# DINT-NSDI24/DINT

Hardware: AMD Instinct MI355X
Metric: Mtxn/s + p50/p99 batch latency, TATP (higher is better)
Workload: dtype u64

## Files before the change

### dint_amd/csrc/dint_bins.h

```cpp
#pragma once
#include <cstdlib>

#include "dint_kernels.h"

#define KV_TB 1024u
#define KV_NONE 0xFFFFFFFFu

__device__ static inline uint32_t block_hash_insert(uint32_t *keys, uint32_t k) {
  uint32_t h = (k * 0x9E3779B1u) >> (32 - 11);
  for (;;) {
    const uint32_t old = atomicCAS(&keys[h], KV_NONE, k);
    if (old == KV_NONE || old == k) return h;
    h = (h + 1) & (2 * KV_TB - 1);
  }
}
static_assert(KV_TB == 1024, "block_hash_insert assumes 2048 slots");

#define KV_PLACE_GRID 64u
__device__ static inline void
kv_scan_place_body(const uint32_t *__restrict__ bin_cnt, uint32_t *bin_off, const uint32_t *__restrict__ big,
                   uint32_t *__restrict__ big_next, uint32_t *__restrict__ blk_pub_next, uint32_t *tail,
                   dint_dev_stats *__restrict__ stats, const uint4 *__restrict__ ovl, uint64_t *__restrict__ ovf) {
  __shared__ uint32_t Sw[KV_TB / 64];
  const uint32_t t = threadIdx.x, lane = t & 63, wave = t >> 6;
  const bool first = blockIdx.x == 0;
  if (first) {
    if (t < 4) big_next[t] = 0;
    blk_pub_next[t] = 0;
    if (t == 0 && tail) tail[0] = tail[1];
  }
  const uint32_t nbig = big[0], novl = big[1];
  if (nbig == 0) return;
  uint32_t run = 0;
  for (uint32_t lo = 0; lo < nbig; lo += KV_TB) {
    const uint32_t bin = lo + t < nbig ? big[4 + lo + t] : KV_NONE;
    const uint32_t extra = bin != KV_NONE ? bin_cnt[bin] - DINT_KV_BINCAP : 0;
    uint32_t tot, x = wave_excl_scan_u32(extra, &tot);
    __syncthreads();
    if (lane == 0) Sw[wave] = tot;
    __syncthreads();
    uint32_t all = 0;
    for (uint32_t w = 0; w < KV_TB / 64; w++) {
      if (w < wave) x += Sw[w];
      all += Sw[w];
    }
    if (bin != KV_NONE) bin_off[bin] = run + x;
    run += all;
  }
  if (first && t == 0) atomicAdd(&stats->big_bin_requests, (unsigned long long)run + (unsigned long long)nbig * DINT_KV_BINCAP);
  __builtin_amdgcn_fence(__ATOMIC_SEQ_CST, "workgroup");
  __syncthreads();
  for (uint32_t i = blockIdx.x * KV_TB + t; i < novl; i += KV_PLACE_GRID * KV_TB) {
    const uint4 o = ovl[i];
    const uint32_t off = __hip_atomic_load(&bin_off[o.z], __ATOMIC_RELAXED, __HIP_MEMORY_SCOPE_WORKGROUP);
    ovf[off + o.w - DINT_KV_BINCAP] = ((uint64_t)o.y << 32) | o.x;
  }
}
static __global__ void __launch_bounds__(KV_TB)
k_kv_scan_place(const uint32_t *__restrict__ bin_cnt, uint32_t *bin_off, const uint32_t *__restrict__ big,
                uint32_t *__restrict__ big_next, uint32_t *__restrict__ blk_pub_next, uint32_t *tail,
                dint_dev_stats *__restrict__ stats, const uint4 *__restrict__ ovl, uint64_t *__restrict__ ovf) {
  kv_scan_place_body(bin_cnt, bin_off, big, big_next, blk_pub_next, tail, stats, ovl, ovf);
}

#define KVB_T 512u
#define KVB_W (KVB_T / 64u)
#define KVB_GRID 512u
#define KVB_NMAX 4096u
#define KVB_NW (KVB_NMAX / 64u)
#define KVB_NBK 2048u
#define KVB_HOT_MIN 256u
#define KVB_HOT_MIN_LOCKS 256u
#define KVB_MMAX 1024u
static_assert(KVB_NW == 64, "the per-word tables are built with one lane per mask word");
static inline uint32_t dint_hot_min(const char *env, uint32_t dflt) {
  const char *v = getenv(env);
  return v && *v ? (uint32_t)strtoul(v, nullptr, 10) : dflt;
}
struct kvb_lead { uint32_t found_link, slot, ver0, la0, lb0; };
struct kvb_carry { uint32_t la, lb, ver; int src; uint32_t miss; };
struct kvb_pop { uint16_t below[KVB_NW + 1]; };
struct kvb_edge { int16_t last[KVB_NW], next[KVB_NW]; };

__device__ static inline void kvb_build_pop(const uint64_t *M, kvb_pop &P) {
  const uint32_t lane = lane_id();
  uint32_t tot;
  const uint32_t x = wave_excl_scan_u32((uint32_t)__popcll(M[lane]), &tot);
  P.below[lane] = (uint16_t)x;
  if (lane == 63) P.below[KVB_NW] = (uint16_t)tot;
}
__device__ static inline void kvb_build_edge(const uint64_t *M, kvb_edge &E) {
  const int lane = (int)lane_id();
  const uint64_t m = M[lane];
  int hi = m ? lane * 64 + 63 - __clzll((long long)m) : -1;
  int lo = m ? lane * 64 + __ffsll((unsigned long long)m) - 1 : 0x7FFF;
#pragma unroll
  for (int d = 1; d < 64; d <<= 1) {
    const int a = __shfl_up(hi, d, 64), b = __shfl_down(lo, d, 64);
    if (lane >= d) hi = max(hi, a);
    if (lane + d < 64) lo = min(lo, b);
  }
  const int a = __shfl_up(hi, 1, 64), b = __shfl_down(lo, 1, 64);
  E.last[lane] = (int16_t)(lane ? a : -1);
  E.next[lane] = (int16_t)((lane == 63 || b == 0x7FFF) ? -1 : b);
}
__device__ static inline bool kvb_bit(const uint64_t *M, uint32_t p) { return (M[p >> 6] >> (p & 63)) & 1ull; }
__device__ static inline uint32_t kvb_below(const uint64_t *M, const kvb_pop &P, uint32_t x) {
  const uint32_t w = x >> 6, r = x & 63;
  return P.below[w] + (r ? (uint32_t)__popcll(M[w] & ((1ull << r) - 1ull)) : 0u);
}
__device__ static inline uint32_t kvb_popc(const uint64_t *M, const kvb_pop &P, uint32_t a, uint32_t b) {
  return a < b ? kvb_below(M, P, b) - kvb_below(M, P, a) : 0u;
}
__device__ static inline int kvb_last(const uint64_t *M, const kvb_edge &E, uint32_t a, uint32_t b) {
  if (a >= b) return -1;
  const uint32_t w = (b - 1) >> 6, r = b & 63;
  const uint64_t m = M[w] & (r ? (1ull << r) - 1ull : ~0ull);
  const int res = m ? (int)(w * 64 + 63 - __clzll((long long)m)) : (int)E.last[w];
  return res >= (int)a ? res : -1;
}
__device__ static inline int kvb_first(const uint64_t *M, const kvb_edge &E, uint32_t a) {
  if (a >= KVB_NMAX) return -1;
  const uint32_t w = a >> 6;
  const uint64_t m = M[w] & (~0ull << (a & 63));
  return m ? (int)(w * 64 + __ffsll((unsigned long long)m) - 1) : (int)E.next[w];
}
__device__ static inline uint32_t kvb_range_popc(const uint64_t *M, uint32_t a, uint32_t b) {
  uint32_t cnt = 0;
  for (uint32_t w = a >> 6; w <= ((b - 1) >> 6) && a < b; w++) {
    uint64_t m = M[w];
    if (w == (a >> 6)) m &= ~0ull << (a & 63);
    if (w == ((b - 1) >> 6) && (b & 63)) m &= (1ull << (b & 63)) - 1ull;
    cnt += (uint32_t)__popcll(m);
  }
  return cnt;
}

__device__ __forceinline__ static uint32_t lane_xor_rt(uint32_t v, uint32_t j) { return (uint32_t)__shfl_xor((int)v, (int)j, 64); }
__device__ __forceinline__ static uint64_t lane_xor_rt(uint64_t v, uint32_t j) {
  return ((uint64_t)lane_xor_rt((uint32_t)(v >> 32), j) << 32) | lane_xor_rt((uint32_t)v, j);
}
#ifdef KVB_SORT_INLINE
#define KVB_SORT_ATTR __forceinline__
#else
#define KVB_SORT_ATTR __attribute__((noinline))
#endif
template <int R, class K>
__device__ KVB_SORT_ATTR static void kvb_sort_blocked_t(K *Sk, uint32_t N) {
// ... 62 lines not shown
```

### dint_amd/csrc/k_kv.hip

```cpp
#include "k_kv_dev.h"

dint_kv_fmt dint_kv_format(uint32_t workload) {
  switch (workload) {
    case DINT_WL_STORE: return {53, 0, 0xFFFFFFFFu, 1, 9, 49, 40};
    case DINT_WL_TATP: return {55, 1, 2, 3, 11, 51, 40};
    default: return {23, 1, 2, 3, 11, 19, 8};
  }
}


static inline uint32_t kv_pick_coarse(uint32_t n, uint32_t load) {
  uint64_t c = ((uint64_t)n + load - 1) / load;
  if (c < 1) c = 1;
  if (c > DINT_KV_CMAX) c = DINT_KV_CMAX;
  return (uint32_t)c;
}
static uint32_t kv_env(const char *name, uint32_t dflt) {
  const char *v = getenv(name);
  return v && *v ? (uint32_t)strtoul(v, nullptr, 10) : dflt;
}
static dint_kv_knobs kv_read_knobs() {
  dint_kv_knobs k;
  k.coarse_load = std::min(8192u, std::max(64u, kv_env("DINT_KV_COARSE_LOAD", KVB_T)));
  k.cap = kv_env("DINT_KV_CAP", 0);
// ... 5 lines not shown
  k.no_split = kv_env("DINT_KV_NO_SPLIT", 0);
  k.split_min = std::max(65u, kv_env("DINT_KV_SPLIT_MIN", 65u));
  k.split_target = std::min(448u, std::max(8u, kv_env("DINT_KV_SPLIT_TARGET", 384u)));
  k.one_big_kernel = kv_env("DINT_KV_ONE_BIG_KERNEL", 0);
  k.no_ahead = kv_env("DINT_KV_NO_AHEAD", 0);
  k.no_fuse = kv_env("DINT_KV_NO_FUSE", 0);
  k.sb_split_min = kv_env("DINT_KV_SB_SPLIT_MIN", 65u);
  k.sb_late_grid = std::max(1u, std::min(KVB_GRID, kv_env("DINT_KV_SB_LATE_GRID", 32u)));
  k.sb_npmax = std::max(2u, std::min(KSB_NPMAX, kv_env("DINT_KV_SB_NPMAX", 128u)));
  k.sb_workers = kv_env("DINT_KV_SB_WORKERS", k.sb_npmax + 2u);
  if (k.sb_workers) k.sb_workers = std::max(k.sb_workers, k.sb_npmax + 2u);
  k.workers = std::min(1024u, std::max(KVR_NPMAX + 2u, kv_env("DINT_KV_WORKERS", KVW_GRID)));
  k.part_first = kv_env("DINT_KV_PART_FIRST", 0) & 1u;
  k.late_grid = std::min(KVB_GRID, std::max(1u, kv_env("DINT_KV_LATE_GRID", 8u)));
  k.late_big = kv_env("DINT_KV_LATE_BIG", 0);
  k.exp_no_late = kv_env("DINT_EXP_NO_LATE", 0);
  k.late_fat = kv_env("DINT_KV_LATE_FAT", 0);
  return k;
}

static inline bool kv_uses_hot(const dint_kv &kv, int load_mode) {
  return kv.workload != DINT_WL_SMALLBANK && !(kv.force_rounds & 3) && !load_mode && !kv.knobs.no_split;
}
bool dint_kv_one_launch(const dint_kv &kv, int load_mode) {
  return kv_uses_hot(kv, load_mode) && !kv.knobs.one_big_kernel && !kv.knobs.no_fuse;
}
bool dint_kv_ahead_ok(const dint_kv &kv, int load_mode) {
  if (kv.workload == DINT_WL_SMALLBANK) return !load_mode && !kv.knobs.no_ahead && !kv.knobs.no_fuse;
  return kv_uses_hot(kv, load_mode) && !kv.knobs.one_big_kernel && !kv.knobs.no_ahead;
}

static void kv_fill_pass(kv_pass_args &A, const void *d_req, void *d_rep, uint32_t n, const dint_kv &kv, dint_log log,
                         const dint_scratch &s, int load_mode, const dint_view &view, uint32_t tile) {
  const dint_kv_knobs &K = kv.knobs;
  const uint32_t C = kv_pick_coarse(n, K.coarse_load);
  const uint32_t mean = (n + C - 1) / C;
  uint32_t cap = K.cap_mult * mean + 64;
  cap = std::min(cap, (uint32_t)(s.kbins_slots / C));
  cap = std::max(1u, K.cap ? std::min(cap, K.cap) : cap);
  A.req = (const uint8_t *)d_req; A.rep = (uint8_t *)d_rep; A.n = n;
  A.n_tiles = (n + tile - 1) / tile;
  A.kv = kv.d_dev; A.log = log; A.cut = kv_make_cut(C, n); A.cap = cap;
  A.lcap = K.lcap;
  const uint64_t pn = s.kvs.pass_no;
  A.pno = (uint32_t)(pn & 1u);
  A.bin_cnt = s.kvs.bin_cnt[pn & 1]; A.kbins = s.kvs.kbins[pn & 1]; A.ovl = s.kvs.ovl[pn & 1];
  A.big = s.kvs.ctl[pn % 3]; A.big_z = s.kvs.ctl[(pn + 2) % 3];
  A.blk_pub = s.kvs.pub[pn % 3]; A.blk_pub_z = s.kvs.pub[(pn + 2) % 3];
  A.bigrdy = s.kvs.bigrdy;
  A.ovf = s.ovf; A.ovf2 = s.ovf2; A.stats = s.stats;
  A.bigq = s.bigq;
  A.hotpub = s.hotpub;
  A.lateq = s.lateq;
  A.seq = s.pass_seq ? s.pass_seq : 1u;
  A.inv_n = n > 1 ? (uint32_t)((1ull << 32) / n) : 0xFFFFFFFFu;
  A.load_mode = load_mode;
  A.force_flags = kv.force_rounds | (K.no_bm ? 4 : 0) | (int)(K.hot_min << 8);
  A.split_min = kv_uses_hot(kv, load_mode) ? K.split_min : 0xFFFFFFFFu;
  A.split_target = K.split_target;
  A.np_max = KVR_NPMAX;
  A.sb_pieces = 0;
  A.sbx = s.kvs.sbx;
  if (kv.workload == DINT_WL_SMALLBANK && K.sb_split_min && s.kvs.sbx && !(kv.force_rounds & 3) && !load_mode && !K.no_split) {
    A.split_min = std::max(8u, K.sb_split_min);
    A.np_max = K.sb_npmax;
    A.sb_pieces = 1;
  }
  A.has_log = kv.workload != DINT_WL_STORE;
  A.trace = kv.d_trace;
  A.V = view;
}

extern template int kv_piece_residency<DINT_WL_STORE>(int);
extern template int kv_piece_residency<DINT_WL_TATP>(int);
extern template int kv_piece_residency<DINT_WL_SMALLBANK>(int);
extern template void launch_kv_passes<DINT_WL_STORE>(kv_multi_args &, uint32_t, uint32_t, hipStream_t, hipEvent_t *, const dint_kv_knobs &, bool, const kv_multi_args *, uint32_t);
extern template void launch_kv_passes<DINT_WL_TATP>(kv_multi_args &, uint32_t, uint32_t, hipStream_t, hipEvent_t *, const dint_kv_knobs &, bool, const kv_multi_args *, uint32_t);
extern template void launch_kv_passes<DINT_WL_SMALLBANK>(kv_multi_args &, uint32_t, uint32_t, hipStream_t, hipEvent_t *, const dint_kv_knobs &, bool, const kv_multi_args *, uint32_t);

static inline uint32_t kv_pick_rpt(uint32_t n_total, const dint_kv_knobs &K) {
  if (K.rpt == 1 || K.rpt == 2 || K.rpt == 4) return K.rpt;
  return n_total >= 1024u * 1024u ? 4u : n_total >= 256u * 1024u ? 2u : 1u;
}
static inline uint32_t kv_pick_rpt_ahead(uint32_t n, const dint_kv_knobs &K) {
  if (K.rpt == 4 || (K.rpt == 0 && n >= 256u * 1024u)) return 4u;
  return 2u;
}

static void launch_kv_dispatch(uint32_t workload, kv_multi_args &M, uint32_t n_eng, uint32_t rpt, hipStream_t st, hipEvent_t *ev,
                               const dint_kv_knobs &K, bool part_done = false, const kv_multi_args *next = nullptr, uint32_t next_rpt = 0) {
  switch (workload) {
    case DINT_WL_STORE: launch_kv_passes<DINT_WL_STORE>(M, n_eng, rpt, st, ev, K, part_done, next, next_rpt); break;
    case DINT_WL_TATP: launch_kv_passes<DINT_WL_TATP>(M, n_eng, rpt, st, ev, K, part_done, next, next_rpt); break;
    default: launch_kv_passes<DINT_WL_SMALLBANK>(M, n_eng, rpt, st, ev, K, part_done, next, next_rpt); break;
  }
}

void dint_launch_kv(const void *d_req, void *d_rep, uint32_t n, const dint_kv &kv, dint_log log, dint_scratch s,
                    int load_mode, hipStream_t st, hipEvent_t *ev, const dint_view &view, bool part_done, const dint_kv_ahead *next) {
  if (n == 0) return;
  kv_multi_args M;
  memset(&M, 0, sizeof M);
  const uint32_t rpt = kv_pick_rpt(n, kv.knobs), rpt_a = kv_pick_rpt_ahead(n, kv.knobs);
  kv_fill_pass(M.e[0], d_req, d_rep, n, kv, log, s, load_mode, view, part_done ? KVB_T * rpt_a : KV_TB * rpt);
  kv_multi_args N;
  uint32_t next_rpt = 0;
  if (next && next->n && dint_kv_ahead_ok(kv, load_mode)) {
    dint_scratch sn = s;
    sn.kvs.pass_no = s.kvs.pass_no + 1;
    sn.pass_seq = s.pass_seq + 1 >= 0x3FFFFFFFu ? 1u : s.pass_seq + 1;
    next_rpt = kv_pick_rpt_ahead(next->n, kv.knobs);
    memset(&N, 0, sizeof N);
    kv_fill_pass(N.e[0], next->d_req, next->d_rep, next->n, kv, log, sn, load_mode, next->view, KVB_T * next_rpt);
  } else {
    next = nullptr;
  }
  launch_kv_dispatch(kv.workload, M, 1, rpt, st, ev, kv.knobs, part_done, next ? &N : nullptr, next_rpt);
}

void dint_launch_kv_multi(const dint_kv_pass *p, uint32_t n_eng, hipStream_t st, bool part_done, const dint_kv_pass *next) {
  if (n_eng == 0) return;
  kv_multi_args M, N;
  memset(&M, 0, sizeof M);
  uint32_t n_total = 0;
  for (uint32_t k = 0; k < n_eng; k++) n_total += p[k].n;
  const uint32_t rpt = kv_pick_rpt(n_total, p[0].kv->knobs);
  for (uint32_t k = 0; k < n_eng; k++) kv_fill_pass(M.e[k], p[k].d_req, p[k].d_rep, p[k].n, *p[k].kv, p[k].log, p[k].s, 0, p[k].view, KV_TB * rpt);
  uint32_t next_rpt = 0;
  if (next) {
    uint32_t nmax = 0;
    for (uint32_t k = 0; k < n_eng; k++) nmax = std::max(nmax, next[k].n);
    next_rpt = kv_pick_rpt_ahead(nmax, p[0].kv->knobs);
    memset(&N, 0, sizeof N);
    for (uint32_t k = 0; k < n_eng; k++) {
      dint_scratch sn = next[k].s;
      sn.kvs.pass_no = p[k].s.kvs.pass_no + 1;
      sn.pass_seq = p[k].s.pass_seq + 1 >= 0x3FFFFFFFu ? 1u : p[k].s.pass_seq + 1;
      kv_fill_pass(N.e[k], next[k].d_req, next[k].d_rep, next[k].n, *next[k].kv, next[k].log, sn, 0, next[k].view, KVB_T * next_rpt);
    }
  }
  launch_kv_dispatch(p[0].kv->workload, M, n_eng, rpt, st, nullptr, p[0].kv->knobs, part_done, next ? &N : nullptr, next_rpt);
}
bool dint_kv_multi_ahead_ok(const dint_kv &kv) { return dint_kv_ahead_ok(kv, 0) && !kv.knobs.no_fuse; }

__global__ void __launch_bounds__(256)
k_home_kv(const uint8_t *__restrict__ req, uint32_t n, const kv_dev *__restrict__ kv, dint_kv_fmt f,
          uint8_t *__restrict__ home) {
  const uint32_t i = blockIdx.x * 256u + threadIdx.x;
  if (i >= n) return;
  const uint8_t *m = req + (size_t)i * f.msg;
  const uint32_t table = f.table == 0xFFFFFFFFu ? 0 : m[f.table];
  if (table >= kv->n_tables) { home[i] = 0xFF; return; }
  const uint64_t g = dint_fastmod(dint_hash_key(ld_u64(m + f.key)), kv->mod[table]);
  home[i] = (uint8_t)(g % (kv->shard_count ? kv->shard_count : 1));
}
void dint_launch_home_kv(const void *d_req, uint32_t n, const dint_kv &kv, uint8_t *d_home, hipStream_t st) {
  if (n == 0) return;
  hipLaunchKernelGGL(k_home_kv, dim3((n + 255) / 256), dim3(256), 0, st, (const uint8_t *)d_req, n, kv.d_dev,
                     dint_kv_format(kv.workload), d_home);
}

int dint_kv_create(dint_kv *kv, uint32_t workload, uint64_t n_rows, dint_shard shard, uint32_t pool_entries,
                   uint32_t flags) {
  *kv = dint_kv();
  kv->workload = workload;
  kv->h.same_key = (workload == DINT_WL_TATP && (flags & DINT_FLAG_LOCK_SAME_KEY)) ? 1 : 0;
  uint64_t hs[DINT_KV_MAX_TABLES] = {0, 0, 0, 0, 0};
  if (workload == DINT_WL_STORE) {
// ... 206 lines not shown
```

### dint_amd/csrc/k_kv_dev.h

```cpp
#pragma once
#include <algorithm>
#include <cstdlib>
#include <cstring>
#include <utility>
#include <vector>

#include "../../include/dint_abi.h"
#include "dint_kv.h"
#define KVB_SORT_INLINE
#include "dint_bins.h"

template <int WL> struct Fmt;
template <> struct Fmt<DINT_WL_STORE> {
  static constexpr uint32_t MSG = 53, TYPE = 0, KEY = 1, VAL = 9, VER = 49, VS = 40;
  static constexpr bool HAS_TABLE = false;
  static constexpr uint32_t TABLE = 0;
};
template <> struct Fmt<DINT_WL_TATP> {
  static constexpr uint32_t MSG = 55, TYPE = 1, KEY = 3, VAL = 11, VER = 51, VS = 40;
  static constexpr bool HAS_TABLE = true;
  static constexpr uint32_t TABLE = 2;
};
template <> struct Fmt<DINT_WL_SMALLBANK> {
  static constexpr uint32_t MSG = 23, TYPE = 1, KEY = 3, VAL = 11, VER = 19, VS = 8;
// ... 69 lines not shown
  uint32_t q = __umulhi(gk, c.magic), r = gk - q * c.P;
  if (r >= c.P) { r -= c.P; q++; }
  *bin = r;
  return q;
}
__device__ static inline uint32_t kv_cut_gk(uint32_t gq, uint32_t bin, const kv_cut &c) { return gq * c.P + bin; }
__device__ static inline uint64_t kv_rec(uint32_t gq, uint32_t idx, uint32_t pay, const kv_cut &c) {
  return ((uint64_t)gq << (16 + c.ibits)) | ((uint64_t)idx << 16) | (pay & 0xFFFFu);
}
__device__ static inline uint32_t kv_rec_pay(uint64_t r) { return (uint32_t)r & 0xFFFFu; }
__device__ static inline uint32_t kv_rec_idx(uint64_t r, const kv_cut &c) { return (uint32_t)(r >> 16) & (uint32_t)((1ull << c.ibits) - 1ull); }
__device__ static inline uint64_t kv_sort_key(uint64_t r, const kv_cut &c) {
  const uint32_t pay = kv_rec_pay(r);
  return ((r >> (16 + c.ibits)) << (16 + c.ibits)) | ((uint64_t)((pay >> 7) & 511u) << (7 + c.ibits)) |
         ((uint64_t)kv_rec_idx(r, c) << 7) | (pay & 0x7Fu);
}

struct kv_reqinfo {
  uint32_t type, table, cls;
  uint64_t key;
};
template <int WL>
__device__ static inline kv_reqinfo kv_read_request(const uint8_t *m, bool live, const kv_dev *kv, int load_mode) {
  using F = Fmt<WL>;
  kv_reqinfo r = {0, 0, 0, 0};
  if (live) {
    r.type = m[F::TYPE];
    r.table = F::HAS_TABLE ? m[F::TABLE] : 0;
    r.cls = kv_class<WL>(r.type, load_mode);
    if (r.table >= kv->n_tables) r.cls = 0;
    if (r.cls) r.key = ld_u64(m + F::KEY);
  }
  return r;
}

struct kv_pass_args {
  const uint8_t *req;
  uint8_t *rep;
  uint32_t n, n_tiles;
  const kv_dev *kv;
  dint_log log;
  kv_cut cut;
  uint32_t cap;
  uint32_t lcap;
  uint32_t *bin_cnt;
  uint4 *kbins;
  uint32_t *big, *big_z;
  uint32_t *blk_pub, *blk_pub_z;
  uint32_t *bigrdy;
  uint64_t *sbx;
  uint32_t np_max;
  uint32_t sb_pieces;
  uint32_t pno;
  uint4 *ovl;
  uint64_t *ovf;
  uint64_t *ovf2;
  uint4 *bigq;
  unsigned long long *hotpub;
  uint4 *lateq;
  uint32_t split_min;
  uint32_t split_target;
  uint32_t inv_n;
  uint32_t seq;
  dint_dev_stats *stats;
  int load_mode, force_flags;
  uint32_t has_log;
  uint64_t *trace;
  dint_view V;
};
struct kv_multi_args { kv_pass_args e[DINT_KV_MULTI_MAX]; };

__device__ static inline uint64_t u4_key(const uint4 &r) { return ((uint64_t)r.y << 32) | r.x; }
__device__ static inline uint64_t u4_meta(const uint4 &r) { return ((uint64_t)r.w << 32) | r.z; }

template <uint32_t TB, uint32_t... Ks>
__device__ __forceinline__ static void kv_copy_tile(const uint4 *__restrict__ s, uint4 *__restrict__ d, uint32_t nv, uint32_t t,
                                                    std::integer_sequence<uint32_t, Ks...>) {
  const uint4 v[] = {s[min(t + Ks * TB, nv - 1)]...};
  ((d[min(t + Ks * TB, nv - 1)] = v[Ks]), ...);
}

template <int RPT, uint32_t TB = KV_TB>
struct kv_part_lds {
  uint32_t Hc[DINT_KV_CMAX];
  uint32_t Sov[2];
  uint32_t Stile;
  uint32_t Swl[TB / 64 * RPT], Swp[TB / 64];
};
template <int WL, int RPT, uint32_t TB = KV_TB>
__device__ __forceinline__ static void kv_part_body(const kv_pass_args &A, kv_part_lds<RPT, TB> &S, bool first_block) {
  using F = Fmt<WL>;
  constexpr uint32_t T = TB * RPT, NWV = TB / 64;
  auto &Hc = S.Hc; auto &Sov = S.Sov; auto &Stile = S.Stile; auto &Swl = S.Swl; auto &Swp = S.Swp;
  const uint32_t t = threadIdx.x, lane = t & 63, wv = t >> 6;
  const uint32_t n = A.n, C = A.cut.P;
  const kv_dev *__restrict__ kv = A.kv;
  const uint8_t *__restrict__ req = A.req;
  uint8_t *rep = A.rep;
  if (t == 0) { Stile = atomicAdd(&A.big[2], 1u); Sov[0] = 0; }
  for (uint32_t k = t; k < C; k += TB) Hc[k] = 0;
  __syncthreads();
  const uint32_t tile = Stile;
  kv_reqinfo r[RPT];
  size_t moff[RPT];
  uint64_t lm[RPT];
  uint32_t idx[RPT];
#pragma unroll
  for (int j = 0; j < RPT; j++) {
    idx[j] = tile * T + (uint32_t)j * TB + t;
    bool live;
    moff[j] = dint_view_off(A.V, idx[j] < n ? idx[j] : 0, F::MSG, &live);
    live = live && idx[j] < n;
    r[j] = kv_read_request<WL>(req + moff[j], live, kv, A.load_mode);
    lm[j] = __ballot(r[j].cls == 2);
    if (live && !r[j].cls) atomicAdd(&A.stats->bad_requests, 1ULL);
  }
  if (WL != DINT_WL_STORE) {
    if (lane == 0) {
#pragma unroll
      for (int j = 0; j < RPT; j++) Swl[j * NWV + wv] = (uint32_t)__popcll(lm[j]);
    }
    __syncthreads();
    if (t == 0) {
      uint32_t c = 0;
      for (uint32_t w = 0; w < NWV * RPT; w++) c += Swl[w];
      __hip_atomic_store(&A.blk_pub[tile], 0x80000000u | c, __ATOMIC_RELAXED, __HIP_MEMORY_SCOPE_AGENT);
    }
  }
  if (rep != req) {
    const size_t lo = (size_t)tile * T * F::MSG;
    const size_t hi = min((size_t)n * F::MSG, lo + (size_t)T * F::MSG);
    if ((((uintptr_t)req | (uintptr_t)rep) & 15) == 0) {
      constexpr uint32_t K = (T * F::MSG / 16 + TB - 1) / TB;
      const uint32_t nv = (uint32_t)((hi - lo) / 16);
      const uint4 *s = (const uint4 *)(req + lo);
      uint4 *d = (uint4 *)(rep + lo);
      if (nv) kv_copy_tile<TB>(s, d, nv, t, std::make_integer_sequence<uint32_t, K>());
      for (size_t k = lo + (size_t)nv * 16 + t; k < hi; k += TB) rep[k] = req[k];
    } else {
      for (size_t k = lo + t; k < hi; k += TB) rep[k] = req[k];
    }
  }

  uint32_t coarse[RPT], mypos[RPT];
  uint64_t meta[RPT];
#pragma unroll
  for (int j = 0; j < RPT; j++) {
    coarse[j] = KV_NONE; mypos[j] = 0; meta[j] = 0;
    if (r[j].cls == 1) {
      const uint64_t h = dint_hash_key(r[j].key);
      const uint64_t g = dint_fastmod(h, kv->mod[r[j].table]);
      uint32_t local = (uint32_t)g;
      bool mine = true;
      if (kv->shard_count > 1) {
        mine = (uint32_t)(g % kv->shard_count) == kv->shard_index;
        if (!mine && !A.load_mode) atomicAdd(&A.stats->foreign_requests, 1ULL);
        local = (uint32_t)(g / kv->shard_count);
      }
      if (mine) {
        const uint64_t hs = kv->mod[r[j].table].d, dq = dint_fastmod(h, kv->lockmod[r[j].table]) - g;
        const uint32_t q = dq >= 2 * hs ? (dq >= 3 * hs ? 3u : 2u) : (dq >= hs ? 1u : 0u);
        const uint32_t gq = kv_cut_div(kv->gk_base[r[j].table] + local, A.cut, &coarse[j]);
        meta[j] = kv_rec(gq, idx[j], kv_pay(r[j].type, q, (uint32_t)(h >> 40) & 511u), A.cut);
        mypos[j] = atomicAdd(&Hc[coarse[j]], 1u);
      }
    }
  }
  __syncthreads();
  for (uint32_t c = t; c < C; c += TB) {
    const uint32_t cnt = Hc[c];
    if (cnt) Hc[c] = atomicAdd(&A.bin_cnt[c], cnt);
  }
  __syncthreads();
  uint32_t orank[RPT];
  bool over[RPT];
#pragma unroll
  for (int j = 0; j < RPT; j++) {
    over[j] = false; orank[j] = 0;
    if (coarse[j] != KV_NONE) {
      const uint32_t pos = Hc[coarse[j]] + mypos[j];
      if (pos < A.cap) {
        A.kbins[(size_t)coarse[j] * A.cap + pos] = make_uint4((uint32_t)r[j].key, (uint32_t)(r[j].key >> 32), (uint32_t)meta[j], (uint32_t)(meta[j] >> 32));
      } else {
        over[j] = true;
        orank[j] = atomicAdd(&Sov[0], 1u);
      }
    }
  }
  __syncthreads();
  if (Sov[0]) {
    if (t == 0) Sov[1] = atomicAdd(&A.big[1], Sov[0]);
    __syncthreads();
#pragma unroll
    for (int j = 0; j < RPT; j++)
      if (over[j]) {
        uint4 *o = A.ovl + 2 * (size_t)(Sov[1] + orank[j]);
        o[0] = make_uint4((uint32_t)r[j].key, (uint32_t)(r[j].key >> 32), (uint32_t)meta[j], (uint32_t)(meta[j] >> 32));
        o[1] = make_uint4(coarse[j], 0u, 0u, 0u);
      }
  }

  if (WL != DINT_WL_STORE) {
    const dint_log log = A.log;
    uint32_t part = 0;
    for (uint32_t k = t; k < tile; k += TB) {
      uint32_t v;
      do { v = __hip_atomic_load(&A.blk_pub[k], __ATOMIC_RELAXED, __HIP_MEMORY_SCOPE_AGENT); } while (!(v >> 31));
      part += v & 0x7FFFFFFFu;
    }
    uint32_t tot;
    wave_excl_scan_u32(part, &tot);
    if (lane == 0) Swp[wv] = tot;
    __syncthreads();
    uint32_t base = 0, tile_total = 0;
    for (uint32_t w = 0; w < NWV; w++) base += Swp[w];
    for (uint32_t w = 0; w < NWV * RPT; w++) tile_total += Swl[w];
    const uint32_t tw = A.pno & 1u;
    if (tile == A.n_tiles - 1 && t == 0) {
      const uint32_t total = base + tile_total;
      log.tail[tw ^ 1u] = (uint32_t)(((uint64_t)log.tail[tw] + total) % log.cap);
      *(unsigned long long *)(log.tail + 2) += total;
    }
#pragma unroll
    for (int j = 0; j < RPT; j++) {
      if (r[j].cls != 2) continue;
      uint32_t pos_in_batch = base + (uint32_t)__popcll(lm[j] & lanemask_lt());
      for (uint32_t w = 0; w < (uint32_t)j * NWV + wv; w++) pos_in_batch += Swl[w];
      const uint32_t pos = (uint32_t)(((uint64_t)log.tail[tw] + pos_in_batch) % log.cap);
      uint8_t *e8 = log.ring + (size_t)pos * 64;
      const uint8_t *m = req + moff[j];
      const uint32_t ver = ld_u32(m + F::VER);
      uint8_t *rp = rep + moff[j];
      if (WL == DINT_WL_TATP && r[j].type == 24) {
        *(uint64_t *)e8 = r[j].key;
        *(uint2 *)(e8 + 48) = make_uint2(ver, 1u | (r[j].table << 8));
        rp[F::TYPE] = 27;
      } else {
        const uint8_t *v8 = m + F::VAL;
        uint4 *e4 = (uint4 *)e8;
        e4[0] = make_uint4((uint32_t)r[j].key, (uint32_t)(r[j].key >> 32), ld_u32(v8), ld_u32(v8 + 4));
        if (F::VS == 40) {
          e4[1] = make_uint4(ld_u32(v8 + 8), ld_u32(v8 + 12), ld_u32(v8 + 16), ld_u32(v8 + 20));
          e4[2] = make_uint4(ld_u32(v8 + 24), ld_u32(v8 + 28), ld_u32(v8 + 32), ld_u32(v8 + 36));
        }
        *(uint2 *)(e8 + 48) = make_uint2(ver, r[j].table << 8);
        rp[F::TYPE] = (WL == DINT_WL_TATP) ? 17 : 15;
      }
    }
  }
  if (first_block && t < KV_NLISTS)
    for (uint32_t k = 0; k < kv->n_tables; k++) kv_pool_rotate<kv_dev_mem>(kv->tab[k], t, (A.pno & 1u) * KV_NLISTS);
}

template <int WL, int RPT>
__global__ void __launch_bounds__(KV_TB) k_kv_part(kv_multi_args M) {
  const kv_pass_args &A = M.e[blockIdx.y];
  if (blockIdx.x >= A.n_tiles) return;
  __shared__ kv_part_lds<RPT> S;
  kv_part_body<WL, RPT>(A, S, blockIdx.x == 0);
}

__device__ static inline void kv_stamp(uint64_t *tr, uint32_t k) {
  if (tr) {
    asm volatile("s_waitcnt vmcnt(0) lgkmcnt(0)" ::: "memory");
    if (lane_id() == 0) tr[k] = __builtin_amdgcn_s_memrealtime();
  }
}
__device__ static inline void kv_stamp_real(uint64_t *tr, uint32_t k) {
  if (tr && lane_id() == 0) tr[k] = __builtin_amdgcn_s_memrealtime();
}

#define KV_POOL_MARGIN 4096u
__device__ static inline uint32_t kv_pool_low(const kv_tab &t) {
  return __hip_atomic_load(t.pool_top, __ATOMIC_RELAXED, __HIP_MEMORY_SCOPE_AGENT) + KV_POOL_MARGIN >= t.pool_cap;
}

template <int WL>
__device__ static inline void kv_do_request(uint8_t *msg, uint32_t type, uint32_t table, uint32_t q, uint64_t bucket,
                                            const kv_dev *kv, dint_dev_stats *__restrict__ stats) {
  using F = Fmt<WL>;
  const kv_tab t = kv->tab[table];
  uint8_t *ie = kv_entry_ptr(t, bucket, KV_INLINE);
  kv_hdr H;
  kv_hdr_load(H, ie);
  uint2 cnt = make_uint2(0, 0);
  if (WL == DINT_WL_SMALLBANK) cnt = *(const uint2 *)(ie + KV_SB_LOCK_OFF + 8 * q);
  const uint64_t key = ld_u64(msg + F::KEY);
  uint8_t *val = msg + F::VAL;

  uint32_t act = KV_ACT_NONE, code = 0, ins_ver = 0;
  bool miss_counts = false;
  int lock_store = -1;
  bool cnt_store = false;
  if (type == DINT_KV_LOAD_OP) {
    act = KV_ACT_INS;
    ins_ver = ld_u32(msg + F::VER);
  } else if (WL == DINT_WL_STORE) {
    switch (type) {
      case 0: act = KV_ACT_GET; break;
      case 1: act = KV_ACT_SET; break;
      default: act = KV_ACT_INS; code = 8; break;
    }
  } else if (WL == DINT_WL_TATP) {
    const uint32_t lk = (H.lockw >> (8 * q)) & 0xFFu;
    switch (type) {
      case 0: act = KV_ACT_GET; break;
      case 1:
        if (lk == 0) { lock_store = 1; code = 7; }
        else code = (kv->same_key && *(const uint64_t *)(ie + KV_OWNER_OFF + 8 * q) == key) ? 28 : 8;
        break;
      case 2: lock_store = 0; code = 9; break;
      case 12: act = KV_ACT_SET; miss_counts = true; lock_store = 0; code = 15; break;
      case 18: act = KV_ACT_INS; lock_store = 0; code = 20; break;
      case 22: act = KV_ACT_DEL; miss_counts = true; lock_store = 0; code = 25; break;
      case 13: act = KV_ACT_SET; miss_counts = true; code = 16; break;
      case 19: act = KV_ACT_INS; code = 21; break;
      default: act = KV_ACT_DEL; miss_counts = true; code = 26; break;
    }
    if (lock_store >= 0 && (uint32_t)lock_store == lk) lock_store = -1;
  } else {
    switch (type) {
      case 0: if (cnt.x == 0) { cnt.y++; cnt_store = true; act = KV_ACT_GET; miss_counts = true; code = 7; } else code = 8; break;
      case 1: if (cnt.x == 0 && cnt.y == 0) { cnt.x++; cnt_store = true; act = KV_ACT_GET; miss_counts = true; code = 9; } else code = 10; break;
      case 2: cnt.y--; cnt_store = true; code = 11; break;
      case 3: cnt.x--; cnt_store = true; code = 12; break;
      case 4: act = KV_ACT_SET; miss_counts = true; code = 13; break;
      case 17: act = KV_ACT_GET; code = 18; break;
      default: act = KV_ACT_SET; miss_counts = true; code = 14; break;
// ... 3129 lines not shown
  const uint32_t t = threadIdx.x;
  if (t < sizeof(kv_dev) / 4) ((uint32_t *)&Skv)[t] = ((const uint32_t *)A.kv)[t];
  __syncthreads();
  kv_dev_pend_set(Skv, A.pno);
  __syncthreads();
  kv_cut cut2 = A.cut;
  cut2.P = A.cut.P * KVR_F;
  if (from_late) {
    for (uint32_t i = blockIdx.x; i < nq; i += gridDim.x) {
      const uint4 d = A.lateq[i];
      const uint64_t *recs = (d.w ? (const uint64_t *)A.ovf2 : A.ovf) + d.y;
      kv_big_bin<WL>(A.rep, A.n, cut2, &Skv, d.x, recs, d.w || !A.ovf2 ? nullptr : A.ovf2 + d.y, d.z, A.stats, A.force_flags, A.V, Lraw, Lbm, nullptr);
    }
    return;
  }
  uint64_t *tr = A.trace ? A.trace + 2048 * 32 + 32 * (size_t)(blockIdx.y * KVB_GRID + blockIdx.x) : nullptr;
  for (bool first = true;; first = false) {
    __syncthreads();
    if (t == 0) Stk = atomicAdd(&A.big[4], 1u);
    __syncthreads();
    const uint32_t i = Stk;
    if (i >= nq) break;
    const uint4 d = A.bigq[KVQ_W * (size_t)i];
    uint32_t src = 0, off = d.y, cnt = d.z;
    uint64_t *ttr = first ? tr : nullptr;
    if (ttr && t == 0) { ttr[0] = __builtin_amdgcn_s_memrealtime(); ttr[2] = d.z; ttr[3] = d.x; ttr[30] = d.w; }
    const uint64_t t_in = tr ? __builtin_amdgcn_s_memrealtime() : 0ull;
    int run = 1;
    if ((d.w & 3u) == KVQ_SOLO && WL != DINT_WL_SMALLBANK)
      run = kv_solo_item<WL>(A.rep, cut2, &Skv, d, A.ovf, A.ovf2, A.stats, A.force_flags & 1, A.V, Lraw, &src, &off, &cnt, ttr);
    else if ((d.w & 3u) != KVQ_SUB && WL == DINT_WL_SMALLBANK)
      run = kv_sb_item<WL>(A.rep, cut2, &Skv, d, A.bigq[KVQ_W * (size_t)i + 1], A.bigq[KVQ_W * (size_t)i + 2], A.ovf, A.ovf2, A.hotpub, A.sbx, A.seq,
                           A.inv_n, A.stats, A.V, Lraw, &src, &off, &cnt);
    else if ((d.w & 3u) != KVQ_SUB)
      run = kv_hot_item<WL>(A.rep, cut2, &Skv, d, A.bigq[KVQ_W * (size_t)i + 1], A.bigq[KVQ_W * (size_t)i + 2], A.ovf, A.ovf2, A.hotpub, A.seq,
                            A.inv_n, A.stats, A.force_flags & 1, A.V, Lraw, &src, &off, &cnt, ttr);
    if (run) {
      const uint64_t *recs = (src ? (const uint64_t *)A.ovf2 : A.ovf) + off;
      kv_big_bin<WL>(A.rep, A.n, cut2, &Skv, d.x, recs, src || !A.ovf2 ? nullptr : A.ovf2 + off, cnt, A.stats, A.force_flags, A.V, Lraw, Lbm, ttr);
    }
    if (ttr && t == 0) ttr[1] = __builtin_amdgcn_s_memrealtime();
    if (tr && t == 0) {
      const uint64_t dt = __builtin_amdgcn_s_memrealtime() - t_in;
      if (dt > (tr[31] >> 40)) tr[31] = (dt << 40) | ((uint64_t)(d.z & 0xFFFFFu) << 20) | (d.w & 0x3FFFFu) | (run ? 1ull << 18 : 0ull);
    }
  }
}

template <int WL>
int kv_piece_residency(int device) {
  int per_cu = 0, cus = 0;
  hipError_t e1 = WL == DINT_WL_SMALLBANK
                      ? hipOccupancyMaxActiveBlocksPerMultiprocessor(&per_cu, k_kv_big<WL>, (int)KVB_T, 0)
                      : hipOccupancyMaxActiveBlocksPerMultiprocessor(&per_cu, k_kv_pass<WL, 0>, (int)KVB_T, 0);
  hipError_t e2 = hipDeviceGetAttribute(&cus, hipDeviceAttributeMultiprocessorCount, device);
  if (e1 != hipSuccess || e2 != hipSuccess) { (void)hipGetLastError(); return 0; }
  return per_cu * cus;
}

template <int WL>
void launch_kv_passes(kv_multi_args &M, uint32_t n_eng, uint32_t rpt, hipStream_t st, hipEvent_t *ev, const dint_kv_knobs &K,
                      bool part_done, const kv_multi_args *next , uint32_t next_rpt) {
  uint32_t max_tiles = 0, sum_c = 0;
  for (uint32_t k = 0; k < n_eng; k++) {
    max_tiles = std::max(max_tiles, M.e[k].n_tiles);
    sum_c += M.e[k].cut.P;
  }
  if (ev) hipEventRecord(ev[0], st);
  if (part_done) {}
  else if (rpt == 1) hipLaunchKernelGGL((k_kv_part<WL, 1>), dim3(max_tiles, n_eng), dim3(KV_TB), 0, st, M);
  else if (rpt == 2) hipLaunchKernelGGL((k_kv_part<WL, 2>), dim3(max_tiles, n_eng), dim3(KV_TB), 0, st, M);
  else hipLaunchKernelGGL((k_kv_part<WL, 4>), dim3(max_tiles, n_eng), dim3(KV_TB), 0, st, M);
  if (ev) hipEventRecord(ev[1], st);
  const bool hot = WL != DINT_WL_SMALLBANK && M.e[0].split_min != 0xFFFFFFFFu && !K.one_big_kernel;
  bool fused = false, one = false;
  uint32_t sb_workers = 0;
  if constexpr (WL != DINT_WL_SMALLBANK) {
    if (hot && !K.no_fuse) {
      uint32_t nmax = 0;
      for (uint32_t k = 0; next && k < n_eng; k++) nmax = std::max(nmax, next->e[k].n_tiles);
      const dim3 g(sum_c + K.workers * n_eng + nmax * n_eng);
      if (!next) hipLaunchKernelGGL((k_kv_pass<WL, 0>), g, dim3(KVB_T), 0, st, M, n_eng, sum_c, M, 0u, K.workers, K.part_first);
      else if (next_rpt == 2) hipLaunchKernelGGL((k_kv_pass<WL, 2>), g, dim3(KVB_T), 0, st, M, n_eng, sum_c, *next, nmax, K.workers, K.part_first);
      else hipLaunchKernelGGL((k_kv_pass<WL, 4>), g, dim3(KVB_T), 0, st, M, n_eng, sum_c, *next, nmax, K.workers, K.part_first);
      one = fused = true;
    }
  } else {
    sb_workers = !K.no_fuse && !K.one_big_kernel && M.e[0].sb_pieces ? K.sb_workers : 0u;
    if ((next || sb_workers) && !K.no_fuse) {
      uint32_t nmax = 0;
      for (uint32_t k = 0; next && k < n_eng; k++) nmax = std::max(nmax, next->e[k].n_tiles);
      const dim3 g(sum_c + sb_workers * n_eng + nmax * n_eng);
      if (!next) hipLaunchKernelGGL((k_kv_pass<WL, 0>), g, dim3(KVB_T), 0, st, M, n_eng, sum_c, M, 0u, sb_workers, 0u);
      else if (next_rpt == 2) hipLaunchKernelGGL((k_kv_pass<WL, 2>), g, dim3(KVB_T), 0, st, M, n_eng, sum_c, *next, nmax, sb_workers, K.part_first);
      else hipLaunchKernelGGL((k_kv_pass<WL, 4>), g, dim3(KVB_T), 0, st, M, n_eng, sum_c, *next, nmax, sb_workers, K.part_first);
      one = true;
    }
  }
  if (!one) hipLaunchKernelGGL((k_kv_resolve<WL>), dim3(sum_c), dim3(KVB_T), 0, st, M, n_eng);
  const bool ev3 = ev && one && WL != DINT_WL_SMALLBANK;
  if (ev) hipEventRecord(ev[2], st);
  if constexpr (WL != DINT_WL_SMALLBANK) {
    if (hot && next && !one && n_eng == 1) {
      const dim3 g(KVB_GRID + next->e[0].n_tiles);
      if (next_rpt == 2) hipLaunchKernelGGL((k_kv_hot_part<WL, 2>), g, dim3(KVB_T), 0, st, M.e[0], next->e[0]);
      else hipLaunchKernelGGL((k_kv_hot_part<WL, 4>), g, dim3(KVB_T), 0, st, M.e[0], next->e[0]);
      fused = true;
    }
  }
  if (hot && !fused) hipLaunchKernelGGL((k_kv_hot<WL>), dim3(KVB_GRID, n_eng), dim3(KVB_T), 0, st, M);
  if (ev && !ev3) hipEventRecord(ev[3], st);
  if constexpr (WL != DINT_WL_SMALLBANK) {
    if (hot && K.exp_no_late == 1) {}
    else if (hot && !K.late_big) {
      for (uint32_t r = 0; r < std::max(1u, K.exp_no_late >> 1); r++)
        if (K.late_fat) hipLaunchKernelGGL((k_kv_late<WL, 2>), dim3(KVL_GRID, n_eng), dim3(KVB_T), 0, st, M, r);
        else hipLaunchKernelGGL((k_kv_late<WL, 4>), dim3(KVL_GRID, n_eng), dim3(KVB_T), 0, st, M, r);
    }
    else hipLaunchKernelGGL((k_kv_big<WL>), dim3(hot ? K.late_grid : KVB_GRID, n_eng), dim3(KVB_T), 0, st, M, hot ? 1u : 0u);
  } else {
    hipLaunchKernelGGL((k_kv_big<WL>), dim3(sb_workers ? K.sb_late_grid : KVB_GRID, n_eng), dim3(KVB_T), 0, st, M, sb_workers ? 1u : 0u);
  }
  if (ev) hipEventRecord(ev3 ? ev[3] : ev[4], st);
}
```

Measured before the change: 3024.

## Stage partition records in LDS, sort locally by bin, and enlarge look-ahead tiles

Restructures the partition body to stage each request's key and packed metadata in shared memory. The records are counting-sorted by coarse bin within the tile, so the writes to global bins become contiguous runs instead of scattered per-thread stores. The request copy is done per sub-tile, interleaved with parsing, and log-entry positions are prefix-scanned once. The look-ahead partition tile grows to 8 rows per thread, and the threshold for choosing it is lowered. This raises LDS use per block and may reduce occupancy, and the log path now re-reads request bytes.

```diff
diff --git a/dint_amd/csrc/dint_bins.h b/dint_amd/csrc/dint_bins.h
--- a/dint_amd/csrc/dint_bins.h
+++ b/dint_amd/csrc/dint_bins.h
@@ -64,6 +64,9 @@
 }
 
 #define KVB_T 512u
+#ifndef KVP_AHEAD_RPT
+#define KVP_AHEAD_RPT 8
+#endif
 #define KVB_W (KVB_T / 64u)
 #define KVB_GRID 512u
 #define KVB_NMAX 4096u
diff --git a/dint_amd/csrc/k_kv.hip b/dint_amd/csrc/k_kv.hip
--- a/dint_amd/csrc/k_kv.hip
+++ b/dint_amd/csrc/k_kv.hip
@@ -111,8 +111,9 @@
   if (K.rpt == 1 || K.rpt == 2 || K.rpt == 4) return K.rpt;
   return n_total >= 1024u * 1024u ? 4u : n_total >= 256u * 1024u ? 2u : 1u;
 }
+#define KVP_AHEAD_MIN (128u * 1024u)
 static inline uint32_t kv_pick_rpt_ahead(uint32_t n, const dint_kv_knobs &K) {
-  if (K.rpt == 4 || (K.rpt == 0 && n >= 256u * 1024u)) return 4u;
+  if (K.rpt == 4 || (K.rpt == 0 && n >= KVP_AHEAD_MIN)) return KVP_AHEAD_RPT;
   return 2u;
 }
 
diff --git a/dint_amd/csrc/k_kv_dev.h b/dint_amd/csrc/k_kv_dev.h
--- a/dint_amd/csrc/k_kv_dev.h
+++ b/dint_amd/csrc/k_kv_dev.h
@@ -175,122 +175,185 @@
 
 template <int RPT, uint32_t TB = KV_TB>
 struct kv_part_lds {
+  uint4 st[TB * RPT];
   uint32_t Hc[DINT_KV_CMAX];
-  uint32_t Sov[2];
+  uint32_t Sov[3];
   uint32_t Stile;
-  uint32_t Swl[TB / 64 * RPT], Swp[TB / 64];
+  uint32_t Swl[TB / 64 * RPT + 1];
+  uint32_t Swp[TB / 64], Ssc[TB / 64];
 };
+#define KVP_NOREC (~0ull)
 template <int WL, int RPT, uint32_t TB = KV_TB>
 __device__ __forceinline__ static void kv_part_body(const kv_pass_args &A, kv_part_lds<RPT, TB> &S, bool first_block) {
   using F = Fmt<WL>;
-  constexpr uint32_t T = TB * RPT, NWV = TB / 64;
+  constexpr int RS = RPT >= 2 ? 2 : 1;
+  static_assert(RPT % RS == 0, "a tile is whole sub-tiles");
+  constexpr uint32_t T = TB * RPT, TS = TB * RS, NWV = TB / 64, CPT = DINT_KV_CMAX / TB;
+  constexpr uint32_t IB = T <= 1024 ? 10 : T <= 2048 ? 11 : T <= 4096 ? 12 : 13;
+  static_assert(T <= 8192 && DINT_KV_CMAX % TB == 0 && (TS * F::MSG) % 16 == 0, "tile shape");
   auto &Hc = S.Hc; auto &Sov = S.Sov; auto &Stile = S.Stile; auto &Swl = S.Swl; auto &Swp = S.Swp;
   const uint32_t t = threadIdx.x, lane = t & 63, wv = t >> 6;
   const uint32_t n = A.n, C = A.cut.P;
   const kv_dev *__restrict__ kv = A.kv;
   const uint8_t *__restrict__ req = A.req;
   uint8_t *rep = A.rep;
-  if (t == 0) { Stile = atomicAdd(&A.big[2], 1u); Sov[0] = 0; }
+  if (t == 0) { Stile = atomicAdd(&A.big[2], 1u); Sov[0] = 0; Sov[2] = 0; }
   for (uint32_t k = t; k < C; k += TB) Hc[k] = 0;
   __syncthreads();
-  const uint32_t tile = Stile;
-  kv_reqinfo r[RPT];
-  size_t moff[RPT];
+  const uint32_t tile = Stile, i0 = tile * T;
   uint64_t lm[RPT];
-  uint32_t idx[RPT];
-#pragma unroll
-  for (int j = 0; j < RPT; j++) {
-    idx[j] = tile * T + (uint32_t)j * TB + t;
-    bool live;
-    moff[j] = dint_view_off(A.V, idx[j] < n ? idx[j] : 0, F::MSG, &live);
-    live = live && idx[j] < n;
-    r[j] = kv_read_request<WL>(req + moff[j], live, kv, A.load_mode);
-    lm[j] = __ballot(r[j].cls == 2);
-    if (live && !r[j].cls) atomicAdd(&A.stats->bad_requests, 1ULL);
-  }
   if (WL != DINT_WL_STORE) {
-    if (lane == 0) {
-#pragma unroll
-      for (int j = 0; j < RPT; j++) Swl[j * NWV + wv] = (uint32_t)__popcll(lm[j]);
+#pragma unroll
+    for (int j = 0; j < RPT; j++) {
+      const uint32_t idx = i0 + (uint32_t)j * TB + t;
+      bool live;
+      const size_t moff = dint_view_off(A.V, idx < n ? idx : 0, F::MSG, &live);
+      live = live && idx < n;
+      bool islog = false;
+      if (live) {
+        const uint8_t *m = req + moff;
+        const uint32_t table = F::HAS_TABLE ? m[F::TABLE] : 0;
+        islog = kv_class<WL>(m[F::TYPE], A.load_mode) == 2 && table < kv->n_tables;
+      }
+      lm[j] = __ballot(islog);
+      if (lane == 0) Swl[j * NWV + wv] = (uint32_t)__popcll(lm[j]);
     }
     __syncthreads();
     if (t == 0) {
       uint32_t c = 0;
-      for (uint32_t w = 0; w < NWV * RPT; w++) c += Swl[w];
+      for (uint32_t w = 0; w < NWV * RPT; w++) { const uint32_t v = Swl[w]; Swl[w] = c; c += v; }
+      Swl[NWV * RPT] = c;
       __hip_atomic_store(&A.blk_pub[tile], 0x80000000u | c, __ATOMIC_RELAXED, __HIP_MEMORY_SCOPE_AGENT);
     }
   }
-  if (rep != req) {
-    const size_t lo = (size_t)tile * T * F::MSG;
-    const size_t hi = min((size_t)n * F::MSG, lo + (size_t)T * F::MSG);
-    if ((((uintptr_t)req | (uintptr_t)rep) & 15) == 0) {
-      constexpr uint32_t K = (T * F::MSG / 16 + TB - 1) / TB;
-      const uint32_t nv = (uint32_t)((hi - lo) / 16);
-      const uint4 *s = (const uint4 *)(req + lo);
-      uint4 *d = (uint4 *)(rep + lo);
-      if (nv) kv_copy_tile<TB>(s, d, nv, t, std::make_integer_sequence<uint32_t, K>());
-      for (size_t k = lo + (size_t)nv * 16 + t; k < hi; k += TB) rep[k] = req[k];
+#pragma unroll 1
+  for (uint32_t s = 0; s < (uint32_t)(RPT / RS); s++) {
+    if (rep != req) {
+      const size_t lo = ((size_t)i0 + (size_t)s * TS) * F::MSG;
+      const size_t hi = min((size_t)n * F::MSG, lo + (size_t)TS * F::MSG);
+      if (lo < hi) {
+        if ((((uintptr_t)req | (uintptr_t)rep) & 15) == 0) {
+          constexpr uint32_t K = (TS * F::MSG / 16 + TB - 1) / TB;
+          const uint32_t nv = (uint32_t)((hi - lo) / 16);
+          const uint4 *sv = (const uint4 *)(req + lo);
+          uint4 *dv = (uint4 *)(rep + lo);
+          if (nv) kv_copy_tile<TB>(sv, dv, nv, t, std::make_integer_sequence<uint32_t, K>());
+          for (size_t k = lo + (size_t)nv * 16 + t; k < hi; k += TB) rep[k] = req[k];
+        } else {
+          for (size_t k = lo + t; k < hi; k += TB) rep[k] = req[k];
+        }
+      }
+    }
+#pragma unroll
+    for (int j = 0; j < RS; j++) {
+      const uint32_t slot = (s * RS + (uint32_t)j) * TB + t, idx = i0 + slot;
+      bool live;
+      const size_t moff = dint_view_off(A.V, idx < n ? idx : 0, F::MSG, &live);
+      live = live && idx < n;
+      const kv_reqinfo r = kv_read_request<WL>(req + moff, live, kv, A.load_mode);
+      if (live && !r.cls) atomicAdd(&A.stats->bad_requests, 1ULL);
+      uint64_t meta = KVP_NOREC;
+      if (r.cls == 1) {
+        const uint64_t h = dint_hash_key(r.key);
+        const uint64_t g = dint_fastmod(h, kv->mod[r.table]);
+        uint32_t local = (uint32_t)g;
+        bool mine = true;
+        if (kv->shard_count > 1) {
+          mine = (uint32_t)(g % kv->shard_count) == kv->shard_index;
+          if (!mine && !A.load_mode) atomicAdd(&A.stats->foreign_requests, 1ULL);
+          local = (uint32_t)(g / kv->shard_count);
+        }
+        if (mine) {
+          const uint64_t hs = kv->mod[r.table].d, dq = dint_fastmod(h, kv->lockmod[r.table]) - g;
+          const uint32_t q = dq >= 2 * hs ? (dq >= 3 * hs ? 3u : 2u) : (dq >= hs ? 1u : 0u);
+          const uint32_t gk = kv->gk_base[r.table] + local;
+          uint32_t coarse;
+          (void)kv_cut_div(gk, A.cut, &coarse);
+          meta = ((uint64_t)gk << (16 + IB)) | ((uint64_t)slot << 16) | (kv_pay(r.type, q, (uint32_t)(h >> 40) & 511u) & 0xFFFFu);
+          atomicAdd(&Hc[coarse], 1u);
+        }
+      }
+      S.st[slot] = make_uint4((uint32_t)r.key, (uint32_t)(r.key >> 32), (uint32_t)meta, (uint32_t)(meta >> 32));
+    }
+  }
+  __syncthreads();
+  const uint32_t q = (C + TB - 1) / TB;
+  uint32_t cnt[CPT], D[CPT], sum = 0;
+#pragma unroll
+  for (uint32_t j = 0; j < CPT; j++) {
+    const uint32_t c = t * q + j;
+    cnt[j] = j < q && c < C ? Hc[c] : 0u;
+    sum += cnt[j];
+  }
+  uint32_t wtot, off = wave_excl_scan_u32(sum, &wtot);
+  if (lane == 0) S.Ssc[wv] = wtot;
+  __syncthreads();
+  uint32_t R = 0;
+  for (uint32_t w = 0; w < NWV; w++) { const uint32_t v = S.Ssc[w]; off += w < wv ? v : 0u; R += v; }
+#pragma unroll
+  for (uint32_t j = 0; j < CPT; j++) {
+    const uint32_t c = t * q + j;
+    D[j] = 0;
+    if (j < q && c < C) {
+      if (cnt[j]) D[j] = atomicAdd(&A.bin_cnt[c], cnt[j]) - off;
+      Hc[c] = off;
+      off += cnt[j];
+    }
+  }
+  __syncthreads();
+  {
+    uint4 rec[RPT];
+    uint32_t dst[RPT];
+#pragma unroll
+    for (int j = 0; j < RPT; j++) {
+      rec[j] = S.st[(uint32_t)j * TB + t];
+      dst[j] = KV_NONE;
+      const uint64_t m = u4_meta(rec[j]);
+      if (m != KVP_NOREC) {
+        uint32_t coarse;
+        (void)kv_cut_div((uint32_t)(m >> (16 + IB)), A.cut, &coarse);
+        dst[j] = atomicAdd(&Hc[coarse], 1u);
+      }
+    }
+    __syncthreads();
+#pragma unroll
+    for (int j = 0; j < RPT; j++)
+      if (dst[j] != KV_NONE) S.st[dst[j]] = rec[j];
+#pragma unroll
+    for (uint32_t j = 0; j < CPT; j++) {
+      const uint32_t c = t * q + j;
+      if (j < q && c < C) Hc[c] = D[j];
+    }
+    __syncthreads();
+  }
+  for (uint32_t k = t; k < R; k += TB) {
+    const uint4 v = S.st[k];
+    const uint64_t m = u4_meta(v);
+    uint32_t coarse;
+    const uint32_t gq = kv_cut_div((uint32_t)(m >> (16 + IB)), A.cut, &coarse);
+    const uint32_t pos = Hc[coarse] + k;
+    if (pos < A.cap) {
+      const uint64_t meta = kv_rec(gq, i0 + ((uint32_t)(m >> 16) & ((1u << IB) - 1u)), (uint32_t)m & 0xFFFFu, A.cut);
+      A.kbins[(size_t)coarse * A.cap + pos] = make_uint4(v.x, v.y, (uint32_t)meta, (uint32_t)(meta >> 32));
     } else {
-      for (size_t k = lo + t; k < hi; k += TB) rep[k] = req[k];
-    }
-  }
-
-  uint32_t coarse[RPT], mypos[RPT];
-  uint64_t meta[RPT];
-#pragma unroll
-  for (int j = 0; j < RPT; j++) {
-    coarse[j] = KV_NONE; mypos[j] = 0; meta[j] = 0;
-    if (r[j].cls == 1) {
-      const uint64_t h = dint_hash_key(r[j].key);
-      const uint64_t g = dint_fastmod(h, kv->mod[r[j].table]);
-      uint32_t local = (uint32_t)g;
-      bool mine = true;
-      if (kv->shard_count > 1) {
-        mine = (uint32_t)(g % kv->shard_count) == kv->shard_index;
-        if (!mine && !A.load_mode) atomicAdd(&A.stats->foreign_requests, 1ULL);
-        local = (uint32_t)(g / kv->shard_count);
-      }
-      if (mine) {
-        const uint64_t hs = kv->mod[r[j].table].d, dq = dint_fastmod(h, kv->lockmod[r[j].table]) - g;
-        const uint32_t q = dq >= 2 * hs ? (dq >= 3 * hs ? 3u : 2u) : (dq >= hs ? 1u : 0u);
-        const uint32_t gq = kv_cut_div(kv->gk_base[r[j].table] + local, A.cut, &coarse[j]);
-        meta[j] = kv_rec(gq, idx[j], kv_pay(r[j].type, q, (uint32_t)(h >> 40) & 511u), A.cut);
-        mypos[j] = atomicAdd(&Hc[coarse[j]], 1u);
-      }
-    }
-  }
-  __syncthreads();
-  for (uint32_t c = t; c < C; c += TB) {
-    const uint32_t cnt = Hc[c];
-    if (cnt) Hc[c] = atomicAdd(&A.bin_cnt[c], cnt);
-  }
-  __syncthreads();
-  uint32_t orank[RPT];
-  bool over[RPT];
-#pragma unroll
-  for (int j = 0; j < RPT; j++) {
-    over[j] = false; orank[j] = 0;
-    if (coarse[j] != KV_NONE) {
-      const uint32_t pos = Hc[coarse[j]] + mypos[j];
-      if (pos < A.cap) {
-        A.kbins[(size_t)coarse[j] * A.cap + pos] = make_uint4((uint32_t)r[j].key, (uint32_t)(r[j].key >> 32), (uint32_t)meta[j], (uint32_t)(meta[j] >> 32));
-      } else {
-        over[j] = true;
-        orank[j] = atomicAdd(&Sov[0], 1u);
-      }
+      atomicAdd(&Sov[0], 1u);
     }
   }
   __syncthreads();
   if (Sov[0]) {
     if (t == 0) Sov[1] = atomicAdd(&A.big[1], Sov[0]);
     __syncthreads();
-#pragma unroll
-    for (int j = 0; j < RPT; j++)
-      if (over[j]) {
-        uint4 *o = A.ovl + 2 * (size_t)(Sov[1] + orank[j]);
-        o[0] = make_uint4((uint32_t)r[j].key, (uint32_t)(r[j].key >> 32), (uint32_t)meta[j], (uint32_t)(meta[j] >> 32));
-        o[1] = make_uint4(coarse[j], 0u, 0u, 0u);
-      }
+    for (uint32_t k = t; k < R; k += TB) {
+      const uint4 v = S.st[k];
+      const uint64_t m = u4_meta(v);
+      uint32_t coarse;
+      const uint32_t gq = kv_cut_div((uint32_t)(m >> (16 + IB)), A.cut, &coarse);
+      if (Hc[coarse] + k < A.cap) continue;
+      const uint64_t meta = kv_rec(gq, i0 + ((uint32_t)(m >> 16) & ((1u << IB) - 1u)), (uint32_t)m & 0xFFFFu, A.cut);
+      uint4 *o = A.ovl + 2 * (size_t)(Sov[1] + atomicAdd(&Sov[2], 1u));
+      o[0] = make_uint4(v.x, v.y, (uint32_t)meta, (uint32_t)(meta >> 32));
+      o[1] = make_uint4(coarse, 0u, 0u, 0u);
+    }
   }
 
   if (WL != DINT_WL_STORE) {
@@ -305,9 +368,9 @@
     wave_excl_scan_u32(part, &tot);
     if (lane == 0) Swp[wv] = tot;
     __syncthreads();
-    uint32_t base = 0, tile_total = 0;
+    uint32_t base = 0;
     for (uint32_t w = 0; w < NWV; w++) base += Swp[w];
-    for (uint32_t w = 0; w < NWV * RPT; w++) tile_total += Swl[w];
+    const uint32_t tile_total = Swl[NWV * RPT];
     const uint32_t tw = A.pno & 1u;
     if (tile == A.n_tiles - 1 && t == 0) {
       const uint32_t total = base + tile_total;
@@ -316,27 +379,29 @@
     }
 #pragma unroll
     for (int j = 0; j < RPT; j++) {
-      if (r[j].cls != 2) continue;
-      uint32_t pos_in_batch = base + (uint32_t)__popcll(lm[j] & lanemask_lt());
-      for (uint32_t w = 0; w < (uint32_t)j * NWV + wv; w++) pos_in_batch += Swl[w];
+      if (!((lm[j] >> lane) & 1ull)) continue;
+      const size_t moff = dint_view_off(A.V, i0 + (uint32_t)j * TB + t, F::MSG);
+      const uint8_t *m = req + moff;
+      const uint32_t type = m[F::TYPE], table = F::HAS_TABLE ? m[F::TABLE] : 0;
+      const uint64_t key = ld_u64(m + F::KEY);
+      const uint32_t pos_in_batch = base + Swl[j * NWV + wv] + (uint32_t)__popcll(lm[j] & lanemask_lt());
       const uint32_t pos = (uint32_t)(((uint64_t)log.tail[tw] + pos_in_batch) % log.cap);
       uint8_t *e8 = log.ring + (size_t)pos * 64;
-      const uint8_t *m = req + moff[j];
       const uint32_t ver = ld_u32(m + F::VER);
-      uint8_t *rp = rep + moff[j];
-      if (WL == DINT_WL_TATP && r[j].type == 24) {
-        *(uint64_t *)e8 = r[j].key;
-        *(uint2 *)(e8 + 48) = make_uint2(ver, 1u | (r[j].table << 8));
+      uint8_t *rp = rep + moff;
+      if (WL == DINT_WL_TATP && type == 24) {
+        *(uint64_t *)e8 = key;
+        *(uint2 *)(e8 + 48) = make_uint2(ver, 1u | (table << 8));
         rp[F::TYPE] = 27;
       } else {
         const uint8_t *v8 = m + F::VAL;
         uint4 *e4 = (uint4 *)e8;
-        e4[0] = make_uint4((uint32_t)r[j].key, (uint32_t)(r[j].key >> 32), ld_u32(v8), ld_u32(v8 + 4));
+        e4[0] = make_uint4((uint32_t)key, (uint32_t)(key >> 32), ld_u32(v8), ld_u32(v8 + 4));
         if (F::VS == 40) {
           e4[1] = make_uint4(ld_u32(v8 + 8), ld_u32(v8 + 12), ld_u32(v8 + 16), ld_u32(v8 + 20));
           e4[2] = make_uint4(ld_u32(v8 + 24), ld_u32(v8 + 28), ld_u32(v8 + 32), ld_u32(v8 + 36));
         }
-        *(uint2 *)(e8 + 48) = make_uint2(ver, r[j].table << 8);
+        *(uint2 *)(e8 + 48) = make_uint2(ver, table << 8);
         rp[F::TYPE] = (WL == DINT_WL_TATP) ? 17 : 15;
       }
     }
@@ -3632,7 +3697,7 @@
       const dim3 g(sum_c + K.workers * n_eng + nmax * n_eng);
       if (!next) hipLaunchKernelGGL((k_kv_pass<WL, 0>), g, dim3(KVB_T), 0, st, M, n_eng, sum_c, M, 0u, K.workers, K.part_first);
       else if (next_rpt == 2) hipLaunchKernelGGL((k_kv_pass<WL, 2>), g, dim3(KVB_T), 0, st, M, n_eng, sum_c, *next, nmax, K.workers, K.part_first);
-      else hipLaunchKernelGGL((k_kv_pass<WL, 4>), g, dim3(KVB_T), 0, st, M, n_eng, sum_c, *next, nmax, K.workers, K.part_first);
+      else hipLaunchKernelGGL((k_kv_pass<WL, KVP_AHEAD_RPT>), g, dim3(KVB_T), 0, st, M, n_eng, sum_c, *next, nmax, K.workers, K.part_first);
       one = fused = true;
     }
   } else {
@@ -3643,7 +3708,7 @@
       const dim3 g(sum_c + sb_workers * n_eng + nmax * n_eng);
       if (!next) hipLaunchKernelGGL((k_kv_pass<WL, 0>), g, dim3(KVB_T), 0, st, M, n_eng, sum_c, M, 0u, sb_workers, 0u);
       else if (next_rpt == 2) hipLaunchKernelGGL((k_kv_pass<WL, 2>), g, dim3(KVB_T), 0, st, M, n_eng, sum_c, *next, nmax, sb_workers, K.part_first);
-      else hipLaunchKernelGGL((k_kv_pass<WL, 4>), g, dim3(KVB_T), 0, st, M, n_eng, sum_c, *next, nmax, sb_workers, K.part_first);
+      else hipLaunchKernelGGL((k_kv_pass<WL, KVP_AHEAD_RPT>), g, dim3(KVB_T), 0, st, M, n_eng, sum_c, *next, nmax, sb_workers, K.part_first);
       one = true;
     }
   }
@@ -3654,7 +3719,7 @@
     if (hot && next && !one && n_eng == 1) {
       const dim3 g(KVB_GRID + next->e[0].n_tiles);
       if (next_rpt == 2) hipLaunchKernelGGL((k_kv_hot_part<WL, 2>), g, dim3(KVB_T), 0, st, M.e[0], next->e[0]);
-      else hipLaunchKernelGGL((k_kv_hot_part<WL, 4>), g, dim3(KVB_T), 0, st, M.e[0], next->e[0]);
+      else hipLaunchKernelGGL((k_kv_hot_part<WL, KVP_AHEAD_RPT>), g, dim3(KVB_T), 0, st, M.e[0], next->e[0]);
       fused = true;
     }
   }
```

Result: slower. 2763 (-8.6%).
